# Fung-Lab/MatDeepLearn

Hardware: AMD Instinct MI355X
Metric: edges/sec training CGCNN on bulk_data (higher is better)
Workload: dtype bf16

## Files before the change

include/mdl_hip.h:

```cpp
#ifndef MDL_HIP_H
#define MDL_HIP_H

#include <stddef.h>
#include <stdint.h>

#ifdef __cplusplus
extern "C" {
#endif

#define MDL_VERSION 100

enum { MDL_F32 = 0, MDL_BF16 = 1 };
enum { MDL_SUM = 0, MDL_MEAN = 1, MDL_MAX = 2 };
enum {
    MDL_OK = 0,
    MDL_E_ARG = -1,
    MDL_E_UNSUPP = -2,
    MDL_E_LAUNCH = -3
};

#define MDL_DTYPE_MASK 0xff
#define MDL_DETERMINISTIC 0x100
#define MDL_K3_PER_WAVE 0x200
#define MDL_K3_EDGE_LANE 0x400
// ... 136 lines not shown
int mdl_loss_fwd_bwd_rows(const float* pred, const float* y, int64_t n, int64_t n_total, int kind, float* loss, float* grad,
                          mdlStream_t stream);

#define MDL_BN_REPLICAS 16
int mdl_bn_sums_rows(void);
int mdl_bn_stats_n(const void* x, float* sums, int64_t N, int C, const int64_t* n_rows_dev, int dtype, mdlStream_t stream);
int mdl_bn_apply_n(const void* x, float* sums, const float* gamma, const float* beta, float* save, float* running_mean,
                   float* running_var, void* y, int64_t N, int C, float eps, float momentum, const int64_t* n_rows_dev,
                   int dtype, mdlStream_t stream);
int mdl_bn_bwd_stats_n(const void* dy, const void* x, const float* save, float* sums, int64_t N, int C,
                       const int64_t* n_rows_dev, int dtype, mdlStream_t stream);
int mdl_bn_bwd_apply_n(const void* dy, const void* x, const float* save, float* sums, const float* gamma, void* dx,
                       int64_t N, int C, const int64_t* n_rows_dev, int dtype, mdlStream_t stream);
int mdl_bn_bwd_apply_relu_n(const void* dy, const void* x, const float* save, float* sums, const float* gamma, void* dx,
                            int64_t N, int C, const int64_t* n_rows_dev, int dtype, mdlStream_t stream);
int mdl_linear_act(const void* x, const void* w, const void* bias, void* out, int64_t N, int K, int M, int act, int dtype,
                   mdlStream_t stream);
int mdl_linear_act_in(const void* x, const void* y, int xact, const void* w, const void* bias, void* out, int64_t N, int K,
                      int M, int act, int dtype, mdlStream_t stream);

int mdl_mlp_head_fwd(const void* x, const void* const* w, const void* const* b, void* const* h, int64_t N, int K0, int NL,
                     const int* M, int dtype, mdlStream_t stream);
int mdl_mlp_head_bwd(const void* x, const void* const* w, const void* const* h, const void* gy, void* dx, float* const* dw,
                     float* const* db, int64_t N, int K0, int NL, const int* M, int dtype, mdlStream_t stream);

int mdl_gru_gates_fwd(const void* gi, const void* gh, const float* h, float* h_out, void* out_lp, int64_t N, int C, int dtype,
                      mdlStream_t stream);
int mdl_gru_gates_bwd(const void* gi, const void* gh, const float* h, const float* g_h, const void* g_lp, void* dgi, void* dgh,
                      float* dh, int64_t N, int C, int dtype, mdlStream_t stream);

// ... 85 lines not shown
```

matdeeplearn_amd/_lib.py:

```python
import ctypes
import os

import torch

HERE = os.path.dirname(os.path.abspath(__file__))
LIB_PATH = os.path.join(HERE, "lib", "libmdl_hip.so")


def use_library(path):
    global LIB_PATH, _lib
    if _lib is not None and os.path.abspath(path) != os.path.abspath(LIB_PATH):
        raise MdlError("use_library(%s): %s is already loaded in this process" % (path, LIB_PATH))
    LIB_PATH = path

MDL_F32, MDL_BF16 = 0, 1
MDL_SUM, MDL_MEAN, MDL_MAX = 0, 1, 2
MDL_DTYPE_MASK, MDL_DETERMINISTIC, MDL_K3_PER_WAVE, MDL_K3_EDGE_LANE = 0xFF, 0x100, 0x200, 0x400
MDL_MLP_F32_IO = 0x2000
MDL_SPLIT_BF16 = 0x1000
MDL_BN_SHIFT_ROW = 0x800
MDL_BN_REPLICAS = 16
REDUCE = {"sum": MDL_SUM, "add": MDL_SUM, "mean": MDL_MEAN, "max": MDL_MAX}

_vp, _i64, _i32, _f32, _sz = ctypes.c_void_p, ctypes.c_int64, ctypes.c_int, ctypes.c_float, ctypes.c_size_t
# ... 56 lines not shown
    "mdl_assemble_batch": (_i32, [_vp] * 20 + [_i32, _i32, _i32, _i32, _i32, _vp]),
    "mdl_assemble_batch_padded": (_i32, [_vp] * 20 + [_i32, _i32, _i32, _i32, _i32, _i64, _i64, _vp, _vp, _vp, _vp, _vp]),
    "mdl_nnconv_msg_fwd": (_i32, [_vp] * 5 + [_i64, _i32, _i32, _i32, _vp]),
    "mdl_nnconv_msg_bwd": (_i32, [_vp] * 7 + [_i64, _i32, _i32, _i32, _vp]),
    "mdl_pad_batch_tail": (_i32, [_vp, _vp, _i32, _i64, _vp, _vp, _vp]),
    "mdl_assemble_transposed": (_i32, [_vp] * 13 + [_i32, _i64, _vp]),
    "mdl_pad_edge_tail": (_i32, [_vp, _vp, _i32, _i64, _i64, _vp, _vp, _vp, _vp, _vp, _vp]),
    "mdl_loss_fwd_bwd": (_i32, [_vp, _vp, _i64, _i32, _vp, _vp, _vp]),
    "mdl_loss_fwd_bwd_rows": (_i32, [_vp, _vp, _i64, _i64, _i32, _vp, _vp, _vp]),
    "mdl_bn_sums_rows": (_i32, []),
    "mdl_bn_stats_n": (_i32, [_vp, _vp, _i64, _i32, _vp, _i32, _vp]),
    "mdl_bn_apply_n": (_i32, [_vp] * 8 + [_i64, _i32, _f32, _f32, _vp, _i32, _vp]),
    "mdl_bn_bwd_stats_n": (_i32, [_vp, _vp, _vp, _vp, _i64, _i32, _vp, _i32, _vp]),
    "mdl_bn_bwd_apply_n": (_i32, [_vp] * 6 + [_i64, _i32, _vp, _i32, _vp]),
    "mdl_bn_bwd_apply_relu_n": (_i32, [_vp] * 6 + [_i64, _i32, _vp, _i32, _vp]),
    "mdl_linear_act": (_i32, [_vp, _vp, _vp, _vp, _i64, _i32, _i32, _i32, _i32, _vp]),
    "mdl_dense_bwd": (_i32, [_vp, _i64, _i32, _vp, _i64, _i32, _vp, _i64, _i32, _vp, _vp, _i64, _i32, _vp, _vp, _vp, _i64, _i32, _vp]),
    "mdl_dense_bwd_ex": (_i32, [_vp, _i64, _i32, _vp, _i64, _i32, _vp, _i64, _i32, _vp, _vp, _i64, _i32, _vp, _vp, _vp, _vp, _i64, _i32, _vp]),
    "mdl_tn_scratch_bytes": (_sz, []),
    "mdl_linear_act_stats": (_i32, [_vp, _vp, _vp, _vp, _vp, _vp, _vp, _vp, _vp, _vp, _i64, _i32, _i32, _i32, _vp, _vp, _i32, _vp]),
    "mdl_linear_act_in": (_i32, [_vp, _vp, _i32, _vp, _vp, _vp, _i64, _i32, _i32, _i32, _i32, _vp]),
    "mdl_ssp_bwd": (_i32, [_vp, _vp, _vp, _i64, _i32, _vp]),
    "mdl_linear_gather_act": (_i32, [_vp] * 10 + [_i64, _i32, _i32, _i32, _i32, _vp]),
    "mdl_linear_wide": (_i32, [_vp, _vp, _vp, _i64, _i32, _i64, _i32, _vp]),
    "mdl_mlp_head_fwd": (_i32, [_vp, _vp, _vp, _vp, _i64, _i32, _i32, _vp, _i32, _vp]),
    "mdl_mlp_head_bwd": (_i32, [_vp, _vp, _vp, _vp, _vp, _vp, _vp, _i64, _i32, _i32, _vp, _i32, _vp]),
    "mdl_gru_gates_fwd": (_i32, [_vp, _vp, _vp, _vp, _vp, _i64, _i32, _i32, _vp]),
    "mdl_gru_gates_bwd": (_i32, [_vp, _vp, _vp, _vp, _vp, _vp, _vp, _vp, _i64, _i32, _i32, _vp]),
    "mdl_gemm_tn": (_i32, [_vp, _i64, _i32, _vp, _i64, _i32, _vp, _i64, _i32, _vp]),
    "mdl_split_bf16": (_i32, [_vp, _vp, _vp, _i64, _vp]),
# ... 86 lines not shown
```

matdeeplearn_amd/csrc/bn.hip:

```cpp
#include "mdl_common.h"

namespace mdl {

constexpr int BN_R = MDL_BN_REPLICAS;

__device__ __forceinline__ void bn_totals(const float* __restrict__ sums, float* tot, int C, float* publish) {
    for (int c = threadIdx.x; c < 2 * C; c += blockDim.x) {
        float v[BN_R];
#pragma unroll
        for (int r = 0; r < BN_R; ++r) v[r] = sums[(size_t)r * 2 * C + c];
        float t = 0.0f;
#pragma unroll
        for (int r = 0; r < BN_R; ++r) t += v[r];
        tot[c] = t;
        if (publish && blockIdx.x == 0) publish[c] = t;
    }
    __syncthreads();
}

template <typename T, int MODE, int W>
__global__ __launch_bounds__(256) void bn_reduce_kernel(const T* __restrict__ a, const T* __restrict__ b,
                                                        const float* __restrict__ save, float* __restrict__ sums,
                                                        int64_t Ncap, int C, const int64_t* __restrict__ n_dev) {
    typedef VecW<T, W> V;
    const int64_t N = n_dev ? max((int64_t)1, min(*n_dev, Ncap)) : Ncap;
    __shared__ float red[2][256 * 8 / 8 * 8];
    const int CG = C / W;
    const int rows_per_block = (int)blockDim.x / CG;
    const int cg = threadIdx.x % CG, rl = threadIdx.x / CG;
    const bool active = rl < rows_per_block;
    float s0[W], s1[W], p0[W], p1[W];
#pragma unroll
    for (int j = 0; j < W; ++j) { s0[j] = 0.0f; s1[j] = 0.0f; }
    if (MODE == 0) {
        V::ld(a + cg * W, p0);
    } else {
#pragma unroll
        for (int j = 0; j < W; ++j) { p0[j] = save[cg * W + j]; p1[j] = save[C + cg * W + j]; }
    }
    if (active) {
// ... 30 lines not shown
        float* dst = sums + (size_t)(blockIdx.x % BN_R) * 2 * C;
        unsafeAtomicAdd(dst + c, t0);
        unsafeAtomicAdd(dst + C + c, t1);
    }
}

template <typename T, int W>
__global__ __launch_bounds__(256) void bn_apply_kernel(const T* __restrict__ x, float* __restrict__ sums,
                                                       const float* __restrict__ gamma, const float* __restrict__ beta,
                                                       float* __restrict__ save, float* __restrict__ run_mean,
                                                       float* __restrict__ run_var, T* __restrict__ y, int64_t Ncap, int C,
                                                       float eps, float momentum, const int64_t* __restrict__ n_dev,
                                                       int shift_row) {
    typedef VecW<T, W> V;
    constexpr int U = 4;
    const int64_t N = n_dev ? max((int64_t)1, min(*n_dev, Ncap)) : Ncap;
    __shared__ float tot[512];
    const int CG = C / W;
    const int cg = threadIdx.x % CG;
    const int64_t total = N * CG;
    const int64_t stride = (int64_t)gridDim.x * blockDim.x;
    int64_t q0 = (int64_t)blockIdx.x * blockDim.x + threadIdx.x;
    float v[U][W];
#pragma unroll
    for (int u = 0; u < U; ++u) V::ld(x + (min(q0 + u * stride, total - 1) / CG) * C + cg * W, v[u]);
    float mean[W], scale[W], shiftv[W], sh[W];
    V::ld(x + cg * W, sh);
    if (shift_row) {
        const float* srow = sums + (size_t)(2 * BN_R + 2) * C;
#pragma unroll
        for (int j = 0; j < W; ++j) sh[j] = srow[cg * W + j];
    }
    bn_totals(sums, tot, C, sums + (size_t)BN_R * 2 * C);
    const float invn = 1.0f / (float)N;
#pragma unroll
    for (int j = 0; j < W; ++j) {
        const int c = cg * W + j;
        const float m1 = tot[c] * invn;
        const float var = fmaxf(tot[C + c] * invn - m1 * m1, 0.0f);
        const float istd = rsqrtf(var + eps);
        mean[j] = sh[j] + m1;
        const float g = gamma ? gamma[c] : 1.0f;
        scale[j] = istd * g;
        shiftv[j] = (beta ? beta[c] : 0.0f) - mean[j] * scale[j];
        if (blockIdx.x == 0 && (int)threadIdx.x < CG) {
            save[c] = mean[j];
            save[C + c] = istd;
            if (run_mean) {
                const float unb = N > 1 ? var * ((float)N / (float)(N - 1)) : var;
                run_mean[c] = (1.0f - momentum) * run_mean[c] + momentum * mean[j];
                run_var[c] = (1.0f - momentum) * run_var[c] + momentum * unb;
            }
        }
    }
    while (true) {
#pragma unroll
        for (int u = 0; u < U; ++u) {
            const int64_t q = q0 + u * stride;
#pragma unroll
            for (int j = 0; j < W; ++j) v[u][j] = v[u][j] * scale[j] + shiftv[j];
            if (q < total) V::st(y + (q / CG) * C + cg * W, v[u]);
        }
        q0 += U * stride;
        if (q0 >= total) break;
#pragma unroll
        for (int u = 0; u < U; ++u) V::ld(x + (min(q0 + u * stride, total - 1) / CG) * C + cg * W, v[u]);
    }
    if (N < Ncap) {
        float z[W];
#pragma unroll
        for (int j = 0; j < W; ++j) z[j] = 0.0f;
        for (int64_t q = total + (int64_t)blockIdx.x * blockDim.x + threadIdx.x; q < Ncap * CG; q += stride)
            V::st(y + (q / CG) * C + cg * W, z);
    }
}

template <typename T, int W, bool MASK = false>
__global__ __launch_bounds__(256) void bn_bwd_apply_kernel(const T* __restrict__ dy, const T* __restrict__ x,
                                                           const float* __restrict__ save, float* __restrict__ sums,
                                                           const float* __restrict__ gamma, T* __restrict__ dx, int64_t Ncap,
                                                           int C, const int64_t* __restrict__ n_dev) {
    typedef VecW<T, W> V;
    constexpr int U = 2;
    const int64_t N = n_dev ? max((int64_t)1, min(*n_dev, Ncap)) : Ncap;
    __shared__ float tot[512];
    const int CG = C / W;
    const int cg = threadIdx.x % CG;
    const int64_t total = N * CG;
    const int64_t stride = (int64_t)gridDim.x * blockDim.x;
    int64_t q0 = (int64_t)blockIdx.x * blockDim.x + threadIdx.x;
    float vd[U][W], vx[U][W];
#pragma unroll
    for (int u = 0; u < U; ++u) {
        const int64_t n = min(q0 + u * stride, total - 1) / CG;
        V::ld(dy + n * C + cg * W, vd[u]);
        V::ld(x + n * C + cg * W, vx[u]);
    }
    bn_totals(sums, tot, C, sums + (size_t)BN_R * 2 * C);
    const float invn = 1.0f / (float)N;
// ... 25 lines not shown
            const int64_t n = min(q0 + u * stride, total - 1) / CG;
            V::ld(dy + n * C + cg * W, vd[u]);
            V::ld(x + n * C + cg * W, vx[u]);
        }
    }
    if (N < Ncap) {
        float z[W];
#pragma unroll
        for (int j = 0; j < W; ++j) z[j] = 0.0f;
        for (int64_t q = total + (int64_t)blockIdx.x * blockDim.x + threadIdx.x; q < Ncap * CG; q += stride)
            V::st(dx + (q / CG) * C + cg * W, z);
    }
}


static int bn_width(int C, int dtype) { return (dtype == MDL_BF16 && C % 8 == 0) ? 8 : 4; }
static int bn_threads(int C, int W) { const int cg = C / W; return 256 / cg * cg; }

static int bn_check(const char* name, int64_t N, int C, int dtype, const void* p) {
    MDL_REQUIRE(dtype == MDL_F32 || dtype == MDL_BF16, MDL_E_UNSUPP, "%s: unsupported dtype %d", name, dtype);
    MDL_REQUIRE(N >= 1 && C >= 4 && C % 4 == 0 && C <= 256, MDL_E_UNSUPP,
                "%s: need N>=1 and C a multiple of 4, C<=256 (got N=%lld C=%d)", name, (long long)N, C);
    MDL_REQUIRE(p && reinterpret_cast<uintptr_t>(p) % (bn_width(C, dtype) * (dtype == MDL_BF16 ? 2 : 4)) == 0, MDL_E_ARG,
                "%s: null or misaligned tensor", name);
    return MDL_OK;
}

static unsigned bn_grid(int64_t N, int C, int W, bool det) {
    if (det) return 1;
    const int rows = 256 / (C / W);
    int64_t g = cdiv(N, (int64_t)rows * 8);
    if (g > 1024) g = 1024;
    return (unsigned)(g < 1 ? 1 : g);
}

}

extern "C" int mdl_bn_sums_rows(void) { return 2 * (MDL_BN_REPLICAS + 1); }

extern "C" int mdl_bn_stats_n(const void* x, float* sums, int64_t N, int C, const int64_t* n_dev, int dtype, mdlStream_t stream) {
    using namespace mdl;
    const bool det = (dtype & MDL_DETERMINISTIC) != 0;
// ... 77 lines not shown
```

matdeeplearn_amd/models/_base.py:

```python
import torch
import torch.nn.functional as F
from torch import nn

from .. import ops
from ..nn import BatchNorm1d, Set2Set, lowp_copies as _lowp


def dense(lin, h, split=False):
    if h.dtype == lin.weight.dtype:
        if split and ops.linear_split_ok(h, lin.weight):
            return ops._LinearSplitTN.apply(h, lin.weight, lin.bias)
        return lin(h)
    return ops.linear(h, lin.weight, lin.bias, _lowp(lin))


def dense_act(lin, h, act, split=False):
    if h.dtype == lin.weight.dtype:
        return getattr(F, act)(dense(lin, h, split))
    return ops.linear_act(h, lin.weight, lin.bias, act, _lowp(lin))


class GraphModel(nn.Module):

    def _begin(self, data, dim1, pre_fc_count, gc_count, pool, pool_order, batch_norm, batch_track_stats, act,
# ... 91 lines not shown

    def _post(self, out, final=False):
        lins = list(self.post_lin_list) + [self.lin_out]
        if out.dtype != self.lin_out.weight.dtype and ops.mlp_head_ok(out, lins, self.act):
            return ops.mlp_head(out, lins, [_lowp(lin) for lin in lins], f32_out=final)
        for lin in self.post_lin_list:
            out = dense_act(lin, out, self.act, split=self.split_products)
        return dense(self.lin_out, out)

    def _pool(self, out, data):
        num_graphs = getattr(data, "num_graphs", None)
        if self.pool == "set2set":
            return self.set2set(out, data.batch, num_graphs)
        return ops.POOLS[self.pool](out, data.batch, num_graphs, seg_index=getattr(data, "pool_index", None))

    def _head(self, out, data):
        if self.pool_order == "early":
            out = self._post(self._pool(out, data).to(out.dtype), final=True)
        else:
            out = self._post(out)
            if self.pool == "set2set":
                out = dense(self.lin_out_2, self._pool(out, data).to(out.dtype))
            else:
                out = self._pool(out, data)
        out = out.float()
        return out.view(-1) if out.shape[1] == 1 else out
```

matdeeplearn_amd/models/cgcnn.py:

```python
import torch
from torch import nn

from .. import ops
from ..nn import CGConv
from ._base import GraphModel


class CGCNN(GraphModel):
    needs_by_source = False

    def __init__(self, data, dim1=64, dim2=64, pre_fc_count=1, gc_count=3, post_fc_count=1,
                 pool="global_mean_pool", pool_order="early", batch_norm="True", batch_track_stats="True",
                 act="relu", dropout_rate=0.0, compute_dtype="fp32", **kwargs):
        super().__init__()
        self._begin(data, dim1, pre_fc_count, gc_count, pool, pool_order, batch_norm, batch_track_stats, act,
                    dropout_rate, compute_dtype)
        for _ in range(gc_count):
            self.conv_list.append(CGConv(self.gc_dim, data.num_edge_features, aggr="mean", batch_norm=False))
            self._add_bn(self.gc_dim)
        self._finish(dim2, post_fc_count, self.gc_dim)

    def forward(self, data):
        x, edge_attr, csr = self._inputs(data)
        out = self._pre(x)
        bn_on = self.batch_norm == "True"
        packs = ops.cgconv_prepack(list(self.conv_list), out.dtype, out.device, want_node=torch.is_grad_enabled()) if out.is_cuda else None
        dist = getattr(data, "dist", None)
        for i, conv in enumerate(self.conv_list):
            prev = self.bn_list[i - 1].bias if (bn_on and i > 0) else None
            out = self._drop(conv(out, None, edge_attr, csr=csr, bn=self.bn_list[i] if bn_on else None, bn_shift=prev,
                                  packed=None if packs is None else packs[i], split=self.split_products, dist=dist))
        return self._head(out, data)
```

matdeeplearn_amd/nn.py:

```python
from torch import nn

from . import ops


class CGConv(nn.Module):

    def __init__(self, channels, dim=0, aggr="add", batch_norm=False, bias=True, **kwargs):
        super().__init__()
        if isinstance(channels, (tuple, list)):
            if channels[0] != channels[1]:
                raise ops.MdlError("CGConv: bipartite channel pairs are not on the reference path")
            channels = channels[0]
        if batch_norm:
            raise ops.MdlError("CGConv(batch_norm=True) is not used by the reference (cgcnn.py:81)")
        self.channels, self.dim, self.aggr = channels, dim, aggr
        self.lin_f = nn.Linear(2 * channels + dim, channels, bias=bias)
        self.lin_s = nn.Linear(2 * channels + dim, channels, bias=bias)
        self.reset_parameters()

    def reset_parameters(self):
        self.lin_f.reset_parameters()
        self.lin_s.reset_parameters()

    def forward(self, x, edge_index, edge_attr=None, csr=None, bn=None, bn_shift=None, packed=None, split=False, dist=None):
# ... 333 lines not shown
        self._sync_counter()
        return super().forward(x)

    def after_cgconv(self, conv, x, edge_index, edge_attr, csr, shift=None, packed=None):
        use_batch_stats = self.training or not self.track_running_stats
        if not (use_batch_stats and self.momentum is not None and self.num_features == x.shape[1] and ops.bn_supported(x)
                and ops.cgconv_bn_stats_ok(x, edge_attr, csr)):
            return None
        rm = rv = None
        if self.training and self.track_running_stats:
            rm, rv = self.running_mean, self.running_var
            self._nbt_pending = getattr(self, "_nbt_pending", 0) + 1
        return ops.cgconv_bn(x, edge_index, edge_attr, conv.lin_f.weight, conv.lin_f.bias, conv.lin_s.weight, conv.lin_s.bias,
                             conv.aggr, csr, self.weight, self.bias, rm, rv, self.eps, self.momentum, shift, packed)

    def after_linear_relu(self, h, weight, bias, lowp=None, gathered=None):
        use_batch_stats = self.training or not self.track_running_stats
        if not (use_batch_stats and self.momentum is not None and ops.linear_relu_bn_ok(h, weight, bias is not None, gathered)):
            return None
        rm = rv = None
        if self.training and self.track_running_stats:
            rm, rv = self.running_mean, self.running_var
            self._nbt_pending = getattr(self, "_nbt_pending", 0) + 1
        return ops.linear_relu_bn(h, weight, bias, lowp, self.weight, self.bias, rm, rv, self.eps, self.momentum, gathered)

    def _save_to_state_dict(self, destination, prefix, keep_vars):
        self._sync_counter()
        super()._save_to_state_dict(destination, prefix, keep_vars)

    def _load_from_state_dict(self, *args, **kwargs):
# ... 3 lines not shown
```

matdeeplearn_amd/ops.py:

```python
import collections
import os

import torch

from . import _lib
from ._lib import MdlError, check, dtype_code, lib, ptr, require_hip, stream

_ACT_CODE = {"relu": 1, "ssp": 2}
_LN2 = 0.6931471805599453


def _f32c(t):
    return None if t is None else t.detach().float().contiguous()


def _stream_key(device):
    return (device.index, torch.cuda.current_stream(device).cuda_stream)


class EdgeCSR:

    __slots__ = ("rowptr", "src", "tgt", "eperm", "N", "E", "_row", "_col", "_t", "_attr", "_tb", "_bal", "partial", "__weakref__")

    def __init__(self, rowptr, src, tgt, eperm, N, E, row=None, col=None):
# ... 500 lines not shown
OPTIONS = {
    "deterministic": ("_DET", "bit-reproducible launch shapes of every atomically accumulating kernel (slow; HIP-vs-HIP tests)"),
    "gmr_dw": ("_GMR_DW", "CFConv backward: dh and dw from one walk over the by-source CSR"),
    "balance": ("_BALANCE", "cost-balanced node ranges for the edge-per-lane CGConv backward (E >= 4e5)"),
    "pad128": ("_PAD128", "C in (96, 128): static 128-channel CGConv kernels on zero-padded rows"),
    "rsrc16": ("_RSRC16", "by-source sums of the CGConv backward in bf16 (packed atomics)"),
    "cg_bn_stats": ("_CG_BN_STATS", "BatchNorm statistics in the CGConv forward's epilogue (measured time-neutral: off)"),
    "direct_grads": ("_DIRECT_GRADS", "K3 / K3c add into the final dW layout (measured slower at small batches: off)"),
    "cfconv_fused": ("_CFCONV_FUSED", "K4: the fused CFConv forward"),
    "cfconv_recompute": ("_CFCONV_RECOMPUTE", "K4b: CFConv backward with the filter recomputed (no per-edge activations)"),
    "tn_colsum": ("_TN_COLSUM", "bias gradients out of the TN GEMM"),
    "dense_bwd": ("_DENSE_BWD", "dX + dW + db of a tall dense layer in one pass"),
    "dense_bwd_wide": ("_DENSE_BWD_WIDE", "... also when both widths exceed 128"),
    "mlp_head": ("_MLP_HEAD", "post-FC head as one launch per direction"),
    "linear_wide": ("_LINEAR_WIDE", "NNConv's Y = x W2r on the streaming kernel"),
    "tn_scratch": ("_TN_SCRATCH", "weight-gradient blocks of the TN products as plain stores + a reduce launch (off: atomics from every workgroup)"),
}


def configure(**kw):
    prev = {}
    g = globals()
    for k, v in kw.items():
        if k not in OPTIONS:
            raise MdlError("ops.configure: unknown option %r (known: %s)" % (k, ", ".join(sorted(OPTIONS))))
        attr = OPTIONS[k][0]
        prev[k] = g[attr]
        g[attr] = bool(v)
    return prev


def options():
    return {k: globals()[a] for k, (a, _) in OPTIONS.items()}


def _dflag():
    return _lib.MDL_DETERMINISTIC if _DET else 0

# ... 1507 lines not shown
            and not (M > 128 and kb > 128) and M % 4 == 0 and x.data_ptr() % 16 == 0 and (gathered is None or len(gathered) <= 3))


def linear_relu_bn(x, weight, bias, lowp, bn_weight, bn_bias, running_mean, running_var, eps, momentum, gathered=None):
    w_lp, b_lp = (lowp if lowp is not None and lowp[0].dtype == x.dtype else (None, None))
    gathered = gathered or []
    idx = [ix if ix.dtype == torch.int32 else ix.to(torch.int32) for _, ix in gathered]
    return _LinearReluBN.apply(x, weight, bias, w_lp, b_lp, bn_weight, bn_bias, running_mean, running_var, eps, momentum, idx,
                               *[t.to(x.dtype) for t, _ in gathered])


def batch_norm_train(x, weight, bias, running_mean, running_var, eps=1e-5, momentum=0.1):
    return _BatchNormTrain.apply(x, weight, bias, running_mean, running_var, eps, momentum)


GRAPH_MAX_NEIGHBORS = 64


def _graph_args(pos, node_ptr, cell, pbc):
    require_hip(pos, node_ptr, cell, pbc)
    if pos.dtype != torch.float64 or pos.dim() != 2 or pos.shape[1] != 3:
        raise MdlError("build_graphs: pos must be [N, 3] float64 (got %s %s)" % (tuple(pos.shape), pos.dtype))
    if node_ptr.dtype != torch.int64 or node_ptr.dim() != 1 or node_ptr.numel() < 2:
        raise MdlError("build_graphs: node_ptr must be [G + 1] int64 with G >= 1")
    G = node_ptr.numel() - 1
    if cell.dtype != torch.float64 or tuple(cell.shape) != (G, 3, 3):
        raise MdlError("build_graphs: cell must be [G, 3, 3] float64 (got %s %s)" % (tuple(cell.shape), cell.dtype))
    if pbc.dim() == 2 and tuple(pbc.shape) == (G, 3):
        pbc = (pbc.to(torch.int32) * torch.tensor([1, 2, 4], dtype=torch.int32, device=pbc.device)).sum(1, dtype=torch.int32)
    if pbc.dtype != torch.int32 or tuple(pbc.shape) != (G,):
# ... 110 lines not shown
```

Baseline: 852.7 million.

## Fold last-layer BatchNorm through early mean/add pooling into fused kernels

Adds fused BatchNorm+pool kernels that accumulate per-graph segment sums alongside the BN statistics in one pass over node features. The normalization is then applied analytically to the pooled sums, so the normalized per-node tensor is never written, and the backward pass runs as a small per-graph sums kernel plus one apply pass. CGCNN's last conv layer takes this path when BN is on, pooling is early mean/add and dropout is zero. Shared BN helpers move into a common header. The cost is extra shared-memory atomics and more code paths for the segment bookkeeping.

After: 854.7 million (median of 2 runs). About the same (+0.2%).

```diff
diff --git a/include/mdl_hip.h b/include/mdl_hip.h
--- a/include/mdl_hip.h
+++ b/include/mdl_hip.h
@@ -174,6 +174,16 @@
                        int64_t N, int C, const int64_t* n_rows_dev, int dtype, mdlStream_t stream);
 int mdl_bn_bwd_apply_relu_n(const void* dy, const void* x, const float* save, float* sums, const float* gamma, void* dx,
                             int64_t N, int C, const int64_t* n_rows_dev, int dtype, mdlStream_t stream);
+int mdl_bn_pool_stats(const void* c, const int32_t* rowptr, const int32_t* seg, float* S, float* sums, int64_t N, int C, int B,
+                      int dtype, mdlStream_t stream);
+int mdl_bn_pool_finalize(const void* c, float* sums, const float* S, const int32_t* rowptr, const float* gamma, const float* beta,
+                         float* save, float* running_mean, float* running_var, void* P, int64_t N, int C, int B, float eps,
+                         float momentum, int reduce, int dtype, mdlStream_t stream);
+int mdl_bn_pool_bwd_sums(const void* dP, const float* S, const int32_t* rowptr, const float* save, float* sums, int B, int C,
+                         int reduce, int dtype, mdlStream_t stream);
+int mdl_bn_pool_bwd_apply(const void* c, const void* dP, const int32_t* seg, const int32_t* rowptr, const float* save,
+                          const float* sums, const float* gamma, void* dc, int64_t N, int C, int B, int reduce, int dtype,
+                          mdlStream_t stream);
 int mdl_linear_act(const void* x, const void* w, const void* bias, void* out, int64_t N, int K, int M, int act, int dtype,
                    mdlStream_t stream);
 int mdl_linear_act_in(const void* x, const void* y, int xact, const void* w, const void* bias, void* out, int64_t N, int K,
diff --git a/matdeeplearn_amd/_lib.py b/matdeeplearn_amd/_lib.py
--- a/matdeeplearn_amd/_lib.py
+++ b/matdeeplearn_amd/_lib.py
@@ -94,6 +94,10 @@
     "mdl_bn_bwd_stats_n": (_i32, [_vp, _vp, _vp, _vp, _i64, _i32, _vp, _i32, _vp]),
     "mdl_bn_bwd_apply_n": (_i32, [_vp] * 6 + [_i64, _i32, _vp, _i32, _vp]),
     "mdl_bn_bwd_apply_relu_n": (_i32, [_vp] * 6 + [_i64, _i32, _vp, _i32, _vp]),
+    "mdl_bn_pool_stats": (_i32, [_vp] * 5 + [_i64, _i32, _i32, _i32, _vp]),
+    "mdl_bn_pool_finalize": (_i32, [_vp] * 10 + [_i64, _i32, _i32, _f32, _f32, _i32, _i32, _vp]),
+    "mdl_bn_pool_bwd_sums": (_i32, [_vp] * 5 + [_i32, _i32, _i32, _i32, _vp]),
+    "mdl_bn_pool_bwd_apply": (_i32, [_vp] * 8 + [_i64, _i32, _i32, _i32, _i32, _vp]),
     "mdl_linear_act": (_i32, [_vp, _vp, _vp, _vp, _i64, _i32, _i32, _i32, _i32, _vp]),
     "mdl_dense_bwd": (_i32, [_vp, _i64, _i32, _vp, _i64, _i32, _vp, _i64, _i32, _vp, _vp, _i64, _i32, _vp, _vp, _vp, _i64, _i32, _vp]),
     "mdl_dense_bwd_ex": (_i32, [_vp, _i64, _i32, _vp, _i64, _i32, _vp, _i64, _i32, _vp, _vp, _i64, _i32, _vp, _vp, _vp, _vp, _i64, _i32, _vp]),
diff --git a/matdeeplearn_amd/csrc/bn.hip b/matdeeplearn_amd/csrc/bn.hip
--- a/matdeeplearn_amd/csrc/bn.hip
+++ b/matdeeplearn_amd/csrc/bn.hip
@@ -1,29 +1,13 @@
-#include "mdl_common.h"
+#include "bn_common.h"
 
 namespace mdl {
-
-constexpr int BN_R = MDL_BN_REPLICAS;
-
-__device__ __forceinline__ void bn_totals(const float* __restrict__ sums, float* tot, int C, float* publish) {
-    for (int c = threadIdx.x; c < 2 * C; c += blockDim.x) {
-        float v[BN_R];
-#pragma unroll
-        for (int r = 0; r < BN_R; ++r) v[r] = sums[(size_t)r * 2 * C + c];
-        float t = 0.0f;
-#pragma unroll
-        for (int r = 0; r < BN_R; ++r) t += v[r];
-        tot[c] = t;
-        if (publish && blockIdx.x == 0) publish[c] = t;
-    }
-    __syncthreads();
-}
 
 template <typename T, int MODE, int W>
 __global__ __launch_bounds__(256) void bn_reduce_kernel(const T* __restrict__ a, const T* __restrict__ b,
                                                         const float* __restrict__ save, float* __restrict__ sums,
                                                         int64_t Ncap, int C, const int64_t* __restrict__ n_dev) {
     typedef VecW<T, W> V;
-    const int64_t N = n_dev ? max((int64_t)1, min(*n_dev, Ncap)) : Ncap;
+    const int64_t N = bn_rows(n_dev, Ncap);
     __shared__ float red[2][256 * 8 / 8 * 8];
     const int CG = C / W;
     const int rows_per_block = (int)blockDim.x / CG;
@@ -84,7 +68,7 @@
                                                        int shift_row) {
     typedef VecW<T, W> V;
     constexpr int U = 4;
-    const int64_t N = n_dev ? max((int64_t)1, min(*n_dev, Ncap)) : Ncap;
+    const int64_t N = bn_rows(n_dev, Ncap);
     __shared__ float tot[512];
     const int CG = C / W;
     const int cg = threadIdx.x % CG;
@@ -106,22 +90,12 @@
 #pragma unroll
     for (int j = 0; j < W; ++j) {
         const int c = cg * W + j;
-        const float m1 = tot[c] * invn;
-        const float var = fmaxf(tot[C + c] * invn - m1 * m1, 0.0f);
-        const float istd = rsqrtf(var + eps);
-        mean[j] = sh[j] + m1;
+        float var, istd;
+        bn_channel_stats(tot, C, c, sh[j], invn, eps, mean[j], var, istd);
         const float g = gamma ? gamma[c] : 1.0f;
         scale[j] = istd * g;
         shiftv[j] = (beta ? beta[c] : 0.0f) - mean[j] * scale[j];
-        if (blockIdx.x == 0 && (int)threadIdx.x < CG) {
-            save[c] = mean[j];
-            save[C + c] = istd;
-            if (run_mean) {
-                const float unb = N > 1 ? var * ((float)N / (float)(N - 1)) : var;
-                run_mean[c] = (1.0f - momentum) * run_mean[c] + momentum * mean[j];
-                run_var[c] = (1.0f - momentum) * run_var[c] + momentum * unb;
-            }
-        }
+        if (blockIdx.x == 0 && (int)threadIdx.x < CG) bn_channel_publish(save, run_mean, run_var, C, c, mean[j], var, istd, N, momentum);
     }
     while (true) {
 #pragma unroll
@@ -152,7 +126,7 @@
                                                            int C, const int64_t* __restrict__ n_dev) {
     typedef VecW<T, W> V;
     constexpr int U = 2;
-    const int64_t N = n_dev ? max((int64_t)1, min(*n_dev, Ncap)) : Ncap;
+    const int64_t N = bn_rows(n_dev, Ncap);
     __shared__ float tot[512];
     const int CG = C / W;
     const int cg = threadIdx.x % CG;
@@ -208,18 +182,6 @@
 }
 
 
-static int bn_width(int C, int dtype) { return (dtype == MDL_BF16 && C % 8 == 0) ? 8 : 4; }
-static int bn_threads(int C, int W) { const int cg = C / W; return 256 / cg * cg; }
-
-static int bn_check(const char* name, int64_t N, int C, int dtype, const void* p) {
-    MDL_REQUIRE(dtype == MDL_F32 || dtype == MDL_BF16, MDL_E_UNSUPP, "%s: unsupported dtype %d", name, dtype);
-    MDL_REQUIRE(N >= 1 && C >= 4 && C % 4 == 0 && C <= 256, MDL_E_UNSUPP,
-                "%s: need N>=1 and C a multiple of 4, C<=256 (got N=%lld C=%d)", name, (long long)N, C);
-    MDL_REQUIRE(p && reinterpret_cast<uintptr_t>(p) % (bn_width(C, dtype) * (dtype == MDL_BF16 ? 2 : 4)) == 0, MDL_E_ARG,
-                "%s: null or misaligned tensor", name);
-    return MDL_OK;
-}
-
 static unsigned bn_grid(int64_t N, int C, int W, bool det) {
     if (det) return 1;
     const int rows = 256 / (C / W);
diff --git a/matdeeplearn_amd/csrc/bn_common.h b/matdeeplearn_amd/csrc/bn_common.h
--- /dev/null
+++ b/matdeeplearn_amd/csrc/bn_common.h
@@ -0,0 +1,58 @@
+#pragma once
+#include "mdl_common.h"
+
+namespace mdl {
+
+constexpr int BN_R = MDL_BN_REPLICAS;
+
+__device__ __forceinline__ int64_t bn_rows(const int64_t* __restrict__ n_dev, int64_t Ncap) {
+    return n_dev ? max((int64_t)1, min(*n_dev, Ncap)) : Ncap;
+}
+
+__device__ __forceinline__ void bn_totals(const float* __restrict__ sums, float* tot, int C, float* publish) {
+    for (int c = threadIdx.x; c < 2 * C; c += blockDim.x) {
+        float v[BN_R];
+#pragma unroll
+        for (int r = 0; r < BN_R; ++r) v[r] = sums[(size_t)r * 2 * C + c];
+        float t = 0.0f;
+#pragma unroll
+        for (int r = 0; r < BN_R; ++r) t += v[r];
+        tot[c] = t;
+        if (publish && blockIdx.x == 0) publish[c] = t;
+    }
+    __syncthreads();
+}
+
+__device__ __forceinline__ void bn_channel_stats(const float* tot, int C, int c, float shift, float invn, float eps,
+                                                 float& mean, float& var, float& istd) {
+    const float m1 = tot[c] * invn;
+    var = fmaxf(tot[C + c] * invn - m1 * m1, 0.0f);
+    istd = rsqrtf(var + eps);
+    mean = shift + m1;
+}
+
+__device__ __forceinline__ void bn_channel_publish(float* __restrict__ save, float* __restrict__ run_mean,
+                                                   float* __restrict__ run_var, int C, int c, float mean, float var, float istd,
+                                                   int64_t N, float momentum) {
+    save[c] = mean;
+    save[C + c] = istd;
+    if (run_mean) {
+        const float unb = N > 1 ? var * ((float)N / (float)(N - 1)) : var;
+        run_mean[c] = (1.0f - momentum) * run_mean[c] + momentum * mean;
+        run_var[c] = (1.0f - momentum) * run_var[c] + momentum * unb;
+    }
+}
+
+static inline int bn_width(int C, int dtype) { return (dtype == MDL_BF16 && C % 8 == 0) ? 8 : 4; }
+static inline int bn_threads(int C, int W) { const int cg = C / W; return 256 / cg * cg; }
+
+static inline int bn_check(const char* name, int64_t N, int C, int dtype, const void* p) {
+    MDL_REQUIRE(dtype == MDL_F32 || dtype == MDL_BF16, MDL_E_UNSUPP, "%s: unsupported dtype %d", name, dtype);
+    MDL_REQUIRE(N >= 1 && C >= 4 && C % 4 == 0 && C <= 256, MDL_E_UNSUPP,
+                "%s: need N>=1 and C a multiple of 4, C<=256 (got N=%lld C=%d)", name, (long long)N, C);
+    MDL_REQUIRE(p && reinterpret_cast<uintptr_t>(p) % (bn_width(C, dtype) * (dtype == MDL_BF16 ? 2 : 4)) == 0, MDL_E_ARG,
+                "%s: null or misaligned tensor", name);
+    return MDL_OK;
+}
+
+}
diff --git a/matdeeplearn_amd/csrc/bn_pool.hip b/matdeeplearn_amd/csrc/bn_pool.hip
--- /dev/null
+++ b/matdeeplearn_amd/csrc/bn_pool.hip
@@ -0,0 +1,362 @@
+#include "bn_common.h"
+
+namespace mdl {
+
+constexpr int BP_K = 4;
+
+__device__ __forceinline__ int64_t pool_rows(const int* __restrict__ rowptr, int B, int64_t Ncap) {
+    return max((int64_t)1, min((int64_t)rowptr[B], Ncap));
+}
+
+template <int W> __device__ __forceinline__ void ld_f32(const float* p, float* v) {
+#pragma unroll
+    for (int k = 0; k < W; k += 4) Vec<float>::ld(p + k, v + k);
+}
+template <int W> __device__ __forceinline__ void st_f32(float* p, const float* v) {
+#pragma unroll
+    for (int k = 0; k < W; k += 4) Vec<float>::st(p + k, v + k);
+}
+
+template <typename T, int W>
+__global__ __launch_bounds__(256) void bn_pool_stats_kernel(const T* __restrict__ c, const int* __restrict__ rowptr,
+                                                            const int* __restrict__ seg, float* __restrict__ S,
+                                                            float* __restrict__ sums, int64_t Ncap, int C, int B) {
+    typedef VecW<T, W> V;
+    constexpr int K = BP_K;
+    __shared__ float acc[256 * K * W];
+    const int64_t N = pool_rows(rowptr, B, Ncap);
+    const int CG = C / W, RL = (int)blockDim.x / CG, ROWS = RL * K;
+    const int cg = threadIdx.x % CG, rl = threadIdx.x / CG;
+    float s0[W], s1[W], sh[W];
+#pragma unroll
+    for (int j = 0; j < W; ++j) { s0[j] = 0.0f; s1[j] = 0.0f; }
+    V::ld(c + cg * W, sh);
+    for (int64_t r0 = (int64_t)blockIdx.x * ROWS; r0 < N; r0 += (int64_t)gridDim.x * ROWS) {
+        const int64_t nb = r0 + rl * K;
+        float v[K][W];
+        int g[K], key[K];
+        bool ok[K], start[K];
+#pragma unroll
+        for (int u = 0; u < K; ++u) {
+            const int64_t n = min(nb + u, N - 1);
+            V::ld(c + n * C + cg * W, v[u]);
+            g[u] = min(max(seg[n], 0), B - 1);
+        }
+#pragma unroll
+        for (int u = 0; u < K; ++u) {
+            const int lr = rl * K + u;
+            ok[u] = nb + u < N;
+            key[u] = (int)min(max((int64_t)rowptr[g[u]] - r0, (int64_t)0), (int64_t)lr);
+            start[u] = ok[u] && key[u] == lr;
+            if (start[u]) {
+#pragma unroll
+                for (int j = 0; j < W; ++j) acc[lr * C + cg * W + j] = 0.0f;
+            }
+        }
+        __syncthreads();
+        float run[W];
+#pragma unroll
+        for (int j = 0; j < W; ++j) run[j] = 0.0f;
+        int cur = key[0];
+#pragma unroll
+        for (int u = 0; u < K; ++u) {
+            if (ok[u]) {
+                if (key[u] != cur) {
+#pragma unroll
+                    for (int j = 0; j < W; ++j) { atomicAdd(&acc[cur * C + cg * W + j], run[j]); run[j] = 0.0f; }
+                    cur = key[u];
+                }
+#pragma unroll
+                for (int j = 0; j < W; ++j) {
+                    const float d = v[u][j] - sh[j];
+                    s0[j] += d;
+                    s1[j] += d * d;
+                    run[j] += d;
+                }
+            }
+        }
+        if (ok[0]) {
+#pragma unroll
+            for (int j = 0; j < W; ++j) atomicAdd(&acc[cur * C + cg * W + j], run[j]);
+        }
+        __syncthreads();
+#pragma unroll
+        for (int u = 0; u < K; ++u) {
+            if (start[u]) {
+                const int lr = rl * K + u;
+                const int64_t first = rowptr[g[u]], end = rowptr[g[u] + 1];
+                float t[W];
+#pragma unroll
+                for (int j = 0; j < W; ++j) t[j] = acc[lr * C + cg * W + j];
+                float* dst = S + (size_t)g[u] * C + cg * W;
+                if (first >= r0 && end <= r0 + ROWS) {
+                    st_f32<W>(dst, t);
+                } else {
+#pragma unroll
+                    for (int j = 0; j < W; ++j) unsafeAtomicAdd(dst + j, t[j]);
+                }
+            }
+        }
+        __syncthreads();
+    }
+    float* red0 = acc;
+    float* red1 = acc + 256 * W;
+#pragma unroll
+    for (int j = 0; j < W; ++j) { red0[threadIdx.x * W + j] = s0[j]; red1[threadIdx.x * W + j] = s1[j]; }
+    __syncthreads();
+    for (int ch = threadIdx.x; ch < C; ch += blockDim.x) {
+        const int gq = ch / W, j = ch % W;
+        double t0 = 0.0, t1 = 0.0;
+        for (int r = 0; r < RL; ++r) { t0 += red0[(r * CG + gq) * W + j]; t1 += red1[(r * CG + gq) * W + j]; }
+        float* dst = sums + (size_t)(blockIdx.x % BN_R) * 2 * C;
+        unsafeAtomicAdd(dst + ch, (float)t0);
+        unsafeAtomicAdd(dst + C + ch, (float)t1);
+    }
+}
+
+template <typename T, int W>
+__global__ __launch_bounds__(256) void bn_pool_finalize_kernel(const T* __restrict__ c, float* __restrict__ sums,
+                                                               const float* __restrict__ S, const int* __restrict__ rowptr,
+                                                               const float* __restrict__ gamma, const float* __restrict__ beta,
+                                                               float* __restrict__ save, float* __restrict__ run_mean,
+                                                               float* __restrict__ run_var, T* __restrict__ P, int64_t Ncap,
+                                                               int C, int B, float eps, float momentum, int mean_pool) {
+    typedef VecW<T, W> V;
+    const int64_t N = pool_rows(rowptr, B, Ncap);
+    __shared__ float tot[512];
+    const int CG = C / W;
+    const int cg = threadIdx.x % CG;
+    float sh[W], scale[W], bias[W], m1[W];
+    V::ld(c + cg * W, sh);
+    bn_totals(sums, tot, C, sums + (size_t)BN_R * 2 * C);
+    const float invn = 1.0f / (float)N;
+#pragma unroll
+    for (int j = 0; j < W; ++j) {
+        const int ch = cg * W + j;
+        float mean, var, istd;
+        bn_channel_stats(tot, C, ch, sh[j], invn, eps, mean, var, istd);
+        scale[j] = istd * (gamma ? gamma[ch] : 1.0f);
+        bias[j] = beta ? beta[ch] : 0.0f;
+        m1[j] = tot[ch] * invn;
+        if (blockIdx.x == 0 && (int)threadIdx.x < CG) {
+            bn_channel_publish(save, run_mean, run_var, C, ch, mean, var, istd, N, momentum);
+            save[2 * C + ch] = m1[j];
+        }
+    }
+    const int64_t stride = (int64_t)gridDim.x * blockDim.x;
+    for (int64_t q = (int64_t)blockIdx.x * blockDim.x + threadIdx.x; q < (int64_t)B * CG; q += stride) {
+        const int64_t gi = q / CG;
+        const int cnt = rowptr[gi + 1] - rowptr[gi];
+        float s[W];
+        ld_f32<W>(S + gi * C + cg * W, s);
+        if (mean_pool) {
+#pragma unroll
+            for (int j = 0; j < W; ++j) s[j] = cnt > 0 ? (s[j] / (float)cnt - m1[j]) * scale[j] + bias[j] : 0.0f;
+        } else {
+#pragma unroll
+            for (int j = 0; j < W; ++j) s[j] = cnt > 0 ? (s[j] - (float)cnt * m1[j]) * scale[j] + (float)cnt * bias[j] : 0.0f;
+        }
+        V::st(P + gi * C + cg * W, s);
+    }
+}
+
+template <typename T, int W>
+__global__ __launch_bounds__(256) void bn_pool_bwd_sums_kernel(const T* __restrict__ dP, const float* __restrict__ S,
+                                                               const int* __restrict__ rowptr, const float* __restrict__ save,
+                                                               float* __restrict__ sums, int B, int C, int mean_pool) {
+    typedef VecW<T, W> V;
+    __shared__ float red[2][256 * W];
+    const int CG = C / W, RL = (int)blockDim.x / CG;
+    const int cg = threadIdx.x % CG, rl = threadIdx.x / CG;
+    float s0[W], s1[W], m1[W], istd[W];
+#pragma unroll
+    for (int j = 0; j < W; ++j) { s0[j] = 0.0f; s1[j] = 0.0f; istd[j] = save[C + cg * W + j]; m1[j] = save[2 * C + cg * W + j]; }
+    for (int64_t gi = (int64_t)blockIdx.x * RL + rl; gi < B; gi += (int64_t)gridDim.x * RL) {
+        const int cnt = rowptr[gi + 1] - rowptr[gi];
+        if (cnt <= 0) continue;
+        float d[W], s[W];
+        V::ld(dP + gi * C + cg * W, d);
+        ld_f32<W>(S + gi * C + cg * W, s);
+        const float fc = (float)cnt;
+        if (mean_pool) {
+#pragma unroll
+            for (int j = 0; j < W; ++j) { s0[j] += d[j]; s1[j] += d[j] * ((s[j] / fc - m1[j]) * istd[j]); }
+        } else {
+#pragma unroll
+            for (int j = 0; j < W; ++j) { s0[j] += fc * d[j]; s1[j] += d[j] * ((s[j] - fc * m1[j]) * istd[j]); }
+        }
+    }
+#pragma unroll
+    for (int j = 0; j < W; ++j) { red[0][threadIdx.x * W + j] = s0[j]; red[1][threadIdx.x * W + j] = s1[j]; }
+    __syncthreads();
+    float* tot = sums + (size_t)BN_R * 2 * C;
+    for (int ch = threadIdx.x; ch < C; ch += blockDim.x) {
+        const int gq = ch / W, j = ch % W;
+        double t0 = 0.0, t1 = 0.0;
+        for (int r = 0; r < RL; ++r) { t0 += red[0][(r * CG + gq) * W + j]; t1 += red[1][(r * CG + gq) * W + j]; }
+        unsafeAtomicAdd(tot + ch, (float)t0);
+        unsafeAtomicAdd(tot + C + ch, (float)t1);
+    }
+}
+
+template <typename T, int W>
+__global__ __launch_bounds__(256) void bn_pool_bwd_apply_kernel(const T* __restrict__ c, const T* __restrict__ dP,
+                                                                const int* __restrict__ seg, const int* __restrict__ rowptr,
+                                                                const float* __restrict__ save, const float* __restrict__ sums,
+                                                                const float* __restrict__ gamma, T* __restrict__ dc,
+                                                                int64_t Ncap, int C, int B, int mean_pool) {
+    typedef VecW<T, W> V;
+    constexpr int U = 4;
+    const int64_t N = pool_rows(rowptr, B, Ncap);
+    const int CG = C / W;
+    const int cg = threadIdx.x % CG;
+    const int64_t total = N * CG;
+    const int64_t stride = (int64_t)gridDim.x * blockDim.x;
+    const float* tot = sums + (size_t)BN_R * 2 * C;
+    const float invn = 1.0f / (float)N;
+    float mean[W], istd[W], k0[W], k1[W], gs[W];
+#pragma unroll
+    for (int j = 0; j < W; ++j) {
+        const int ch = cg * W + j;
+        mean[j] = save[ch];
+        istd[j] = save[C + ch];
+        gs[j] = (gamma ? gamma[ch] : 1.0f) * istd[j];
+        k0[j] = tot[ch] * invn;
+        k1[j] = tot[C + ch] * invn;
+    }
+    for (int64_t q0 = (int64_t)blockIdx.x * blockDim.x + threadIdx.x; q0 < total; q0 += U * stride) {
+        float vx[U][W], vd[U][W], sc[U];
+        int gi[U];
+#pragma unroll
+        for (int u = 0; u < U; ++u) {
+            const int64_t n = min(q0 + u * stride, total - 1) / CG;
+            V::ld(c + n * C + cg * W, vx[u]);
+            gi[u] = min(max(seg[n], 0), B - 1);
+        }
+#pragma unroll
+        for (int u = 0; u < U; ++u) {
+            V::ld(dP + (size_t)gi[u] * C + cg * W, vd[u]);
+            sc[u] = mean_pool ? (float)max(rowptr[gi[u] + 1] - rowptr[gi[u]], 1) : 1.0f;
+        }
+#pragma unroll
+        for (int u = 0; u < U; ++u) {
+            const int64_t q = q0 + u * stride;
+#pragma unroll
+            for (int j = 0; j < W; ++j) {
+                const float dy = mean_pool ? vd[u][j] / sc[u] : vd[u][j];
+                vd[u][j] = gs[j] * (dy - k0[j] - (vx[u][j] - mean[j]) * istd[j] * k1[j]);
+            }
+            if (q < total) V::st(dc + (q / CG) * C + cg * W, vd[u]);
+        }
+    }
+    if (N < Ncap) {
+        float z[W];
+#pragma unroll
+        for (int j = 0; j < W; ++j) z[j] = 0.0f;
+        for (int64_t q = total + (int64_t)blockIdx.x * blockDim.x + threadIdx.x; q < Ncap * CG; q += stride)
+            V::st(dc + (q / CG) * C + cg * W, z);
+    }
+}
+
+static int bn_pool_check(const char* name, int64_t N, int C, int B, int reduce, int dtype, const void* rows, const void* graph_rows,
+                         const void* graph_f32, const int32_t* rowptr) {
+    int rc = bn_check(name, N, C, dtype, rows);
+    if (rc) return rc;
+    MDL_REQUIRE(B >= 1 && rowptr, MDL_E_ARG, "%s: need B >= 1 graphs and their row pointers", name);
+    MDL_REQUIRE(reduce == MDL_SUM || reduce == MDL_MEAN, MDL_E_UNSUPP, "%s: sum or mean pooling (got %d)", name, reduce);
+    const uintptr_t es = dtype == MDL_BF16 ? 2 : 4;
+    MDL_REQUIRE(reinterpret_cast<uintptr_t>(graph_rows) % (bn_width(C, dtype) * es) == 0 &&
+                reinterpret_cast<uintptr_t>(graph_f32) % 16 == 0, MDL_E_ARG, "%s: misaligned graph rows", name);
+    return MDL_OK;
+}
+
+#define BN_POOL_LAUNCH(kernel, grid, threads, st, ...)                                                        \
+    do {                                                                                                      \
+        if (dtype == MDL_BF16 && W == 8) {                                                                    \
+            typedef const bf16_t* tp; typedef bf16_t* tq;                                                     \
+            hipLaunchKernelGGL((kernel<bf16_t, 8>), dim3(grid), dim3(threads), 0, st, __VA_ARGS__);           \
+        } else if (dtype == MDL_BF16) {                                                                       \
+            typedef const bf16_t* tp; typedef bf16_t* tq;                                                     \
+            hipLaunchKernelGGL((kernel<bf16_t, 4>), dim3(grid), dim3(threads), 0, st, __VA_ARGS__);           \
+        } else {                                                                                              \
+            typedef const float* tp; typedef float* tq;                                                       \
+            hipLaunchKernelGGL((kernel<float, 4>), dim3(grid), dim3(threads), 0, st, __VA_ARGS__);            \
+        }                                                                                                     \
+    } while (0)
+
+}
+
+extern "C" int mdl_bn_pool_stats(const void* c, const int32_t* rowptr, const int32_t* seg, float* S, float* sums, int64_t N, int C,
+                                 int B, int dtype, mdlStream_t stream) {
+    using namespace mdl;
+    const bool det = (dtype & MDL_DETERMINISTIC) != 0;
+    dtype &= MDL_DTYPE_MASK;
+    int rc = bn_pool_check("mdl_bn_pool_stats", N, C, B, MDL_SUM, dtype, c, nullptr, S, rowptr);
+    if (rc) return rc;
+    MDL_REQUIRE(seg && S && sums, MDL_E_ARG, "mdl_bn_pool_stats: null argument");
+    const int W = bn_width(C, dtype);
+    const unsigned threads = det ? (unsigned)(C / W) : (unsigned)bn_threads(C, W);
+    const int64_t ranges = cdiv(N, (int64_t)(threads / (C / W)) * BP_K);
+    const unsigned grid = det ? 1u : (unsigned)cdiv(ranges, cdiv(ranges, 2048));
+    hipStream_t st = (hipStream_t)stream;
+    BN_POOL_LAUNCH(bn_pool_stats_kernel, grid, threads, st, (tp)c, rowptr, seg, S, sums, N, C, B);
+    return check_launch("mdl_bn_pool_stats");
+}
+
+extern "C" int mdl_bn_pool_finalize(const void* c, float* sums, const float* S, const int32_t* rowptr, const float* gamma,
+                                    const float* beta, float* save, float* running_mean, float* running_var, void* P, int64_t N,
+                                    int C, int B, float eps, float momentum, int reduce, int dtype, mdlStream_t stream) {
+    using namespace mdl;
+    dtype &= MDL_DTYPE_MASK;
+    int rc = bn_pool_check("mdl_bn_pool_finalize", N, C, B, reduce, dtype, c, P, S, rowptr);
+    if (rc) return rc;
+    MDL_REQUIRE(sums && S && save && P, MDL_E_ARG, "mdl_bn_pool_finalize: null argument");
+    const int W = bn_width(C, dtype);
+    int64_t g = cdiv((int64_t)B * (C / W), 256 * 4);
+    if (g > 768) g = 768;
+    const unsigned grid = (unsigned)(g < 1 ? 1 : g), threads = (unsigned)bn_threads(C, W);
+    const int mean_pool = reduce == MDL_MEAN;
+    hipStream_t st = (hipStream_t)stream;
+    BN_POOL_LAUNCH(bn_pool_finalize_kernel, grid, threads, st, (tp)c, sums, S, rowptr, gamma, beta, save, running_mean,
+                   running_var, (tq)P, N, C, B, eps, momentum, mean_pool);
+    return check_launch("mdl_bn_pool_finalize");
+}
+
+extern "C" int mdl_bn_pool_bwd_sums(const void* dP, const float* S, const int32_t* rowptr, const float* save, float* sums, int B,
+                                    int C, int reduce, int dtype, mdlStream_t stream) {
+    using namespace mdl;
+    const bool det = (dtype & MDL_DETERMINISTIC) != 0;
+    dtype &= MDL_DTYPE_MASK;
+    int rc = bn_pool_check("mdl_bn_pool_bwd_sums", B, C, B, reduce, dtype, dP, dP, S, rowptr);
+    if (rc) return rc;
+    MDL_REQUIRE(S && save && sums, MDL_E_ARG, "mdl_bn_pool_bwd_sums: null argument");
+    const int W = bn_width(C, dtype);
+    const unsigned threads = (unsigned)bn_threads(C, W);
+    int64_t g = cdiv(B, (int64_t)(threads / (C / W)) * 2);
+    if (g > 128) g = 128;
+    const unsigned grid = det ? 1u : (unsigned)(g < 1 ? 1 : g);
+    const int mean_pool = reduce == MDL_MEAN;
+    hipStream_t st = (hipStream_t)stream;
+    BN_POOL_LAUNCH(bn_pool_bwd_sums_kernel, grid, threads, st, (tp)dP, S, rowptr, save, sums, B, C, mean_pool);
+    return check_launch("mdl_bn_pool_bwd_sums");
+}
+
+extern "C" int mdl_bn_pool_bwd_apply(const void* c, const void* dP, const int32_t* seg, const int32_t* rowptr, const float* save,
+                                     const float* sums, const float* gamma, void* dc, int64_t N, int C, int B, int reduce, int dtype,
+                                     mdlStream_t stream) {
+    using namespace mdl;
+    dtype &= MDL_DTYPE_MASK;
+    int rc = bn_pool_check("mdl_bn_pool_bwd_apply", N, C, B, reduce, dtype, c, dP, sums, rowptr);
+    if (rc) return rc;
+    MDL_REQUIRE(dP && seg && save && sums && dc, MDL_E_ARG, "mdl_bn_pool_bwd_apply: null argument");
+    MDL_REQUIRE(reinterpret_cast<uintptr_t>(dc) % 16 == 0, MDL_E_ARG, "mdl_bn_pool_bwd_apply: misaligned gradient rows");
+    const int W = bn_width(C, dtype);
+    int64_t g = cdiv(N * (C / W), 256 * 4);
+    if (g > 4096) g = 4096;
+    const unsigned grid = (unsigned)(g < 1 ? 1 : g), threads = (unsigned)bn_threads(C, W);
+    const int mean_pool = reduce == MDL_MEAN;
+    hipStream_t st = (hipStream_t)stream;
+    BN_POOL_LAUNCH(bn_pool_bwd_apply_kernel, grid, threads, st, (tp)c, (tp)dP, seg, rowptr, save, sums, gamma,
+                   (tq)dc, N, C, B, mean_pool);
+    return check_launch("mdl_bn_pool_bwd_apply");
+}
diff --git a/matdeeplearn_amd/models/_base.py b/matdeeplearn_amd/models/_base.py
--- a/matdeeplearn_amd/models/_base.py
+++ b/matdeeplearn_amd/models/_base.py
@@ -129,7 +129,23 @@
             return self.set2set(out, data.batch, num_graphs)
         return ops.POOLS[self.pool](out, data.batch, num_graphs, seg_index=getattr(data, "pool_index", None))
 
-    def _head(self, out, data):
+    _POOL_REDUCE = {"global_mean_pool": "mean", "global_add_pool": "sum"}
+
+    def _bn_pool_index(self, out, data):
+        if not (self.batch_norm == "True" and self.pool_order == "early" and self.pool in self._POOL_REDUCE and self.training
+                and self.dropout_rate == 0.0 and torch.is_tensor(out) and out.is_cuda and len(self.bn_list) > 0):
+            return None
+        si = ops.pool_seg_index(data.batch, getattr(data, "num_graphs", None), getattr(data, "pool_index", None))
+        return si if self.bn_list[-1].pool_ok(out, si, self._POOL_REDUCE[self.pool]) else None
+
+    def _head(self, out, data, bn_pool=None):
+        if bn_pool is not None:
+            bn, si = bn_pool
+            if bn.pool_ok(out, si, self._POOL_REDUCE[self.pool]):
+                out = self._post(bn.then_pool(out, si, self._POOL_REDUCE[self.pool]), final=True)
+                out = out.float()
+                return out.view(-1) if out.shape[1] == 1 else out
+            out = self._drop(bn(out))
         if self.pool_order == "early":
             out = self._post(self._pool(out, data).to(out.dtype), final=True)
         else:
diff --git a/matdeeplearn_amd/models/cgcnn.py b/matdeeplearn_amd/models/cgcnn.py
--- a/matdeeplearn_amd/models/cgcnn.py
+++ b/matdeeplearn_amd/models/cgcnn.py
@@ -26,7 +26,12 @@
         bn_on = self.batch_norm == "True"
         packs = ops.cgconv_prepack(list(self.conv_list), out.dtype, out.device, want_node=torch.is_grad_enabled()) if out.is_cuda else None
         dist = getattr(data, "dist", None)
+        last = len(self.conv_list) - 1
+        si = self._bn_pool_index(out, data) if (bn_on and dist is None) else None
         for i, conv in enumerate(self.conv_list):
+            if i == last and si is not None:
+                out = conv(out, None, edge_attr, csr=csr, packed=None if packs is None else packs[i], split=self.split_products)
+                return self._head(out, data, bn_pool=(self.bn_list[i], si))
             prev = self.bn_list[i - 1].bias if (bn_on and i > 0) else None
             out = self._drop(conv(out, None, edge_attr, csr=csr, bn=self.bn_list[i] if bn_on else None, bn_shift=prev,
                                   packed=None if packs is None else packs[i], split=self.split_products, dist=dist))
diff --git a/matdeeplearn_amd/nn.py b/matdeeplearn_amd/nn.py
--- a/matdeeplearn_amd/nn.py
+++ b/matdeeplearn_amd/nn.py
@@ -371,6 +371,17 @@
         return ops.cgconv_bn(x, edge_index, edge_attr, conv.lin_f.weight, conv.lin_f.bias, conv.lin_s.weight, conv.lin_s.bias,
                              conv.aggr, csr, self.weight, self.bias, rm, rv, self.eps, self.momentum, shift, packed)
 
+    def pool_ok(self, c, seg_index, reduce):
+        return bool(self.training and self.momentum is not None and c.dim() == 2 and self.num_features == c.shape[1]
+                    and ops.bn_pool_ok(c, seg_index, reduce))
+
+    def then_pool(self, c, seg_index, reduce):
+        rm = rv = None
+        if self.track_running_stats:
+            rm, rv = self.running_mean, self.running_var
+            self._nbt_pending = getattr(self, "_nbt_pending", 0) + 1
+        return ops.bn_pool(c, self.weight, self.bias, rm, rv, self.eps, self.momentum, seg_index, reduce)
+
     def after_linear_relu(self, h, weight, bias, lowp=None, gathered=None):
         use_batch_stats = self.training or not self.track_running_stats
         if not (use_batch_stats and self.momentum is not None and ops.linear_relu_bn_ok(h, weight, bias is not None, gathered)):
diff --git a/matdeeplearn_amd/ops.py b/matdeeplearn_amd/ops.py
--- a/matdeeplearn_amd/ops.py
+++ b/matdeeplearn_amd/ops.py
@@ -538,6 +538,7 @@
     "dense_bwd_wide": ("_DENSE_BWD_WIDE", "... also when both widths exceed 128"),
     "mlp_head": ("_MLP_HEAD", "post-FC head as one launch per direction"),
     "linear_wide": ("_LINEAR_WIDE", "NNConv's Y = x W2r on the streaming kernel"),
+    "bn_pool": ("_BN_POOL", "early mean / add pooling behind a training-mode BatchNorm as one node, the BatchNorm folded through the pool"),
     "tn_scratch": ("_TN_SCRATCH", "weight-gradient blocks of the TN products as plain stores + a reduce launch (off: atomics from every workgroup)"),
 }
 
@@ -546,6 +547,7 @@
     prev = {}
     g = globals()
     for k, v in kw.items():
+        k = k.lower()
         if k not in OPTIONS:
             raise MdlError("ops.configure: unknown option %r (known: %s)" % (k, ", ".join(sorted(OPTIONS))))
         attr = OPTIONS[k][0]
@@ -2083,6 +2085,74 @@
     return _BatchNormTrain.apply(x, weight, bias, running_mean, running_var, eps, momentum)
 
 
+_BN_POOL = True
+
+
+def pool_seg_index(batch, size=None, seg_index=None):
+    if seg_index is not None:
+        return seg_index
+    if size is None or not batch.is_cuda:
+        return None
+    return _seg_index(batch, size, True)
+
+
+def bn_pool_ok(c, seg_index, reduce):
+    si = seg_index
+    return bool(_BN_POOL and reduce in ("mean", "sum", "add") and si is not None and si.perm is None and si.N >= 1
+                and c.is_cuda and bn_supported(c) and si.E == c.shape[0] and si.seg.dtype == torch.int32
+                and si.rowptr.dtype == torch.int32 and si.rowptr.numel() == si.N + 1)
+
+
+class _BatchNormPool(torch.autograd.Function):
+
+    @staticmethod
+    def forward(ctx, c, weight, bias, running_mean, running_var, eps, momentum, si, reduce):
+        N, C = c.shape
+        B = si.N
+        dt = dtype_code(c)
+        R = lib().mdl_bn_sums_rows()
+        buf = _zeros_step((R + 3, C), c.device)
+        sums, save = buf[:R], buf[-3:]
+        S = _zeros_step((B, C), c.device)
+        gw, gb = _f32c(weight), _f32c(bias)
+        P = torch.empty((B, C), dtype=c.dtype, device=c.device)
+        check(lib().mdl_bn_pool_stats(ptr(c), ptr(si.rowptr), ptr(si.seg), ptr(S), ptr(sums), N, C, B, dt | _dflag(), stream()),
+              "mdl_bn_pool_stats")
+        check(lib().mdl_bn_pool_finalize(ptr(c), ptr(sums), ptr(S), ptr(si.rowptr), ptr(gw), ptr(gb), ptr(save), ptr(running_mean),
+                                         ptr(running_var), ptr(P), N, C, B, float(eps), float(momentum), reduce, dt, stream()),
+              "mdl_bn_pool_finalize")
+        ctx.save_for_backward(c, S, save, gw)
+        ctx.si, ctx.reduce = si, reduce
+        ctx.has = (weight is not None, bias is not None)
+        ctx.wdt = None if weight is None else weight.dtype
+        return P
+
+    @staticmethod
+    def backward(ctx, dP):
+        c, S, save, gw = ctx.saved_tensors
+        si = ctx.si
+        N, C = c.shape
+        dP = dP.contiguous()
+        dt = dtype_code(c)
+        R = lib().mdl_bn_sums_rows()
+        sums = _zeros_grad(R * C, c.device).view(R, C)
+        dc = torch.empty_like(c)
+        check(lib().mdl_bn_pool_bwd_sums(ptr(dP), ptr(S), ptr(si.rowptr), ptr(save), ptr(sums), si.N, C, ctx.reduce, dt | _dflag(),
+                                         stream()), "mdl_bn_pool_bwd_sums")
+        check(lib().mdl_bn_pool_bwd_apply(ptr(c), ptr(dP), ptr(si.seg), ptr(si.rowptr), ptr(save), ptr(sums), ptr(gw), ptr(dc), N, C,
+                                          si.N, ctx.reduce, dt, stream()), "mdl_bn_pool_bwd_apply")
+        dgamma = sums[R - 1].to(ctx.wdt) if ctx.has[0] else None
+        dbeta = sums[R - 2].to(ctx.wdt) if ctx.has[1] else None
+        return dc, dgamma, dbeta, None, None, None, None, None, None
+
+
+def bn_pool(c, weight, bias, running_mean, running_var, eps, momentum, seg_index, reduce="mean"):
+    require_hip(c)
+    if not bn_pool_ok(c, seg_index, reduce):
+        raise MdlError("ops.bn_pool: operands outside the fused path (check ops.bn_pool_ok first)")
+    return _BatchNormPool.apply(c, weight, bias, running_mean, running_var, eps, momentum, seg_index, _lib.REDUCE[reduce])
+
+
 GRAPH_MAX_NEIGHBORS = 64
 
 
```
